# fakufaku/diffusion-separation

Hardware: AMD Instinct MI355X
Metric: separated utterances/sec (4 s, 8 kHz, 2-spk, N=30 PC steps) (higher is better)
Workload: dtype f16; 1 GPU; configs[1]: 2-spk N=30 PC sampler (+1 ald2 corrector step), batch=16 x 4.0 s @ 8 kHz per GPU and step, NCSN++ nf=64 random-init, 60 NFE/step; 4 consecutive steps (batches) in flight per GPU; batch_per_gpu=16, samples=32000, N=30, corrector_steps=1, nf=64, graph=True, batches_in_flight=4

## Files before the change

### diffusion-separation_amd/csrc/stft.hip

```cpp
#include <math.h>

#include <string.h>

#include <type_traits>
#include <vector>

#include "common.h"

#define DS_MAXC 4

long ds_stft_fwd_offset(int n_fft) { return ((long)3 * n_fft + 63) & ~63L; }
long ds_stft_inv_offset(int n_fft) { return ds_stft_fwd_offset(n_fft) + 512L * 512L; }
long ds_stft_ffrag_offset(int n_fft) { return ds_stft_inv_offset(n_fft) + 512L * 512L; }
constexpr long DS_STFT_FFRAG_FLOATS = 2L * 16 * 32 * 64 * 8 / 2;
long ds_stft_ifrag_offset(int n_fft) { return ds_stft_ffrag_offset(n_fft) + DS_STFT_FFRAG_FLOATS; }
int ds_build_stft_table(int n_fft, float** dev_tab) {
  if (n_fft > 510 || n_fft % 2) { ds_set_error("stft: n_fft must be even and <= 510"); return 1; }
  const int bins = n_fft / 2 + 1;
  std::vector<float> t((size_t)ds_stft_ifrag_offset(n_fft) + DS_STFT_FFRAG_FLOATS, 0.f);
  for (int n = 0; n < n_fft; ++n) {
    const double a = 2.0 * M_PI * (double)n / (double)n_fft;
    t[n] = (float)cos(a);
    t[n_fft + n] = (float)sin(a);
    t[2 * n_fft + n] = (float)(0.5 * (1.0 - cos(a)));
  }
  float* fw = t.data() + ds_stft_fwd_offset(n_fft);
  float* iv = t.data() + ds_stft_inv_offset(n_fft);
  for (int k = 0; k < bins; ++k)
    for (int n = 0; n < n_fft; ++n) {
      const double a = 2.0 * M_PI * (double)(((long)k * n) % n_fft) / (double)n_fft;
      fw[(size_t)k * 512 + n] = (float)cos(a);
      fw[(size_t)(256 + k) * 512 + n] = (float)(-sin(a));
      const double cj = (k == 0 || k == bins - 1) ? 1.0 : 2.0;
      const double wn = 0.5 * (1.0 - cos(2.0 * M_PI * (double)n / (double)n_fft)) / (double)n_fft;
      iv[(size_t)n * 512 + k] = (float)(wn * cj * cos(a));
      iv[(size_t)n * 512 + 256 + k] = (k == 0 || k == bins - 1) ? 0.f : (float)(-wn * cj * sin(a));
    }
  {
    bf16_t* fr = reinterpret_cast<bf16_t*>(t.data() + ds_stft_ffrag_offset(n_fft));
    const size_t part = (size_t)16 * 32 * 64 * 8;
    for (int rt = 0; rt < 16; ++rt)
      for (int ks = 0; ks < 32; ++ks)
        for (int lane = 0; lane < 64; ++lane)
          for (int j = 0; j < 8; ++j) {
            const int r = rt * 32 + (lane & 31), kb = r >> 1, im = r & 1, n = 16 * ks + 8 * (lane >> 5) + j;
            float v = 0.f;
            if (n < n_fft && kb < bins) {
              const double a = 2.0 * M_PI * (double)(((long)kb * n) % n_fft) / (double)n_fft;
              const double wn = 0.5 * (1.0 - cos(2.0 * M_PI * (double)n / (double)n_fft));
              v = (float)(wn * (im ? -sin(a) : cos(a)));
            }
            const bf16_t hi = f2bf(v);
            const size_t o = (((size_t)ks * 16 + rt) * 64 + lane) * 8 + j;
            fr[o] = hi;
            fr[part + o] = f2bf(v - bf2f(hi));
          }
  }
  {
    bf16_t* fr = reinterpret_cast<bf16_t*>(t.data() + ds_stft_ifrag_offset(n_fft));
    const size_t part = (size_t)16 * 32 * 64 * 8;
    for (int ct = 0; ct < 16; ++ct)
      for (int ks = 0; ks < 32; ++ks)
        for (int lane = 0; lane < 64; ++lane)
          for (int j = 0; j < 8; ++j) {
            const int n = ct * 32 + (lane & 31), K = 16 * ks + 8 * (lane >> 5) + j;
            const float v = iv[(size_t)n * 512 + K];
            const bf16_t hi = f2bf(v);
            const size_t o = (((size_t)ks * 16 + ct) * 64 + lane) * 8 + j;
            fr[o] = hi;
            fr[part + o] = f2bf(v - bf2f(hi));
          }
  }
  float* d = nullptr;
  DS_HIP(hipMalloc(&d, t.size() * sizeof(float)));
  DS_HIP(hipMemcpy(d, t.data(), t.size() * sizeof(float), hipMemcpyHostToDevice));
  *dev_tab = d;
  return 0;
}

__global__ __launch_bounds__(256) void stft_frame_kernel(const float* __restrict__ xt, const float* __restrict__ mix,
                                                         float* __restrict__ frames, int S, long Tlen, int n_fft,
                                                         int hop, int F, long rows, const float* __restrict__ tab) {
  const long i = (long)blockIdx.x * 256 + threadIdx.x;
  if (i >= rows * 128) return;
  const long row = i >> 7;
  const int n0 = (int)(i & 127) * 4;
  const int f = (int)(row % F);
  const long bc = row / F;
  const int NC = S + 1;
  const int ch = (int)(bc % NC);
  const long b = bc / NC;
  const float* src = (ch < S) ? xt + (b * S + ch) * Tlen : mix + b * Tlen;
  const long base = (long)f * hop - n_fft / 2;
  float v[4];
#pragma unroll
  for (int j = 0; j < 4; ++j) {
    const int n = n0 + j;
    const long idx = base + n;
    v[j] = (n < n_fft && idx >= 0 && idx < Tlen) ? src[idx] * tab[2 * n_fft + n] : 0.f;
  }
  *reinterpret_cast<float4*>(frames + row * 512 + n0) = make_float4(v[0], v[1], v[2], v[3]);
}

template <typename T>
__global__ __launch_bounds__(256) void stft_pack_kernel(const float* __restrict__ specT, T* __restrict__ y, int S,
                                                        int bins, int F, int W, int Cpad, long rows, float expo,
                                                        float factor, int shift, int B) {
  const long i = (long)blockIdx.x * 256 + threadIdx.x;
  const long total = (long)B * bins * W;
  if (i >= total) return;
  const int f = (int)(i % W);
  const int k = (int)((i / W) % bins);
  const long b = i / ((long)W * bins);
  const int NC = S + 1;
  float o[16];
#pragma unroll
  for (int j = 0; j < 16; ++j) o[j] = 0.f;
  if (f < F) {
#pragma unroll
    for (int ch = 0; ch < DS_MAXC; ++ch) {
      if (ch < NC) {
        const long row = (b * NC + ch) * F + f;
        const float re = specT[(long)k * rows + row], im = specT[(long)(256 + k) * rows + row];
        const float mag = sqrtf(re * re + im * im);
        float sc = 0.f;
        if (mag > 0.f) sc = (expo == 0.5f) ? (1.0f / sqrtf(mag)) : ((expo == 1.0f) ? 1.0f : powf(mag, expo - 1.0f));
        sc *= factor;
        float vr = re * sc, vi = im * sc;
        if (shift) { vr = 2.f * vr - 1.f; vi = 2.f * vi - 1.f; }
        if (ch == 0) { o[0] = vr; }
        if (ch == 1) { o[1] = vr; }
        if (ch == 2) { o[2] = vr; }
        if (ch == 3) { o[3] = vr; }
        const int q = NC + ch;
        if (q == 1) o[1] = vi; else if (q == 2) o[2] = vi; else if (q == 3) o[3] = vi; else if (q == 4) o[4] = vi;
        else if (q == 5) o[5] = vi; else if (q == 6) o[6] = vi; else if (q == 7) o[7] = vi;
      }
    }
  } else {
    const float pv = shift ? -1.f : 0.f;
#pragma unroll
    for (int j = 0; j < 16; ++j) o[j] = (j < 2 * NC) ? pv : 0.f;
  }
  T* dst = y + ((b * bins + k) * W + f) * Cpad;
  for (int c0 = 0; c0 < Cpad; c0 += 8) store8<T>(dst + c0, o + c0);
}

#ifdef ST_TIMING
__device__ unsigned long long g_st_dbg[16];
#define ST_DECL unsigned long long st_prev = __builtin_readcyclecounter();
#define ST_MARK(i) { const unsigned long long st_now = __builtin_readcyclecounter(); if (threadIdx.x == 0) atomicAdd(&g_st_dbg[i], st_now - st_prev); st_prev = st_now; }
extern "C" int diffsep_st_debug_read(unsigned long long* out, int reset) {
  (void)hipMemcpyFromSymbol(out, HIP_SYMBOL(g_st_dbg), sizeof(unsigned long long) * 16);
  if (reset) { unsigned long long z[16] = {0}; (void)hipMemcpyToSymbol(HIP_SYMBOL(g_st_dbg), z, sizeof(z)); }
  return 0;
}
#else
#define ST_DECL
#define ST_MARK(i)
#endif
constexpr int SF_PITCH = 272, SF_ROWS = 35, SF_CH = SF_ROWS * SF_PITCH, SF_NS = 32 * 128 + 382;
#ifndef SF_NW
#define SF_NW 4
#endif
constexpr int SF_NT = 64 * SF_NW, SF_RT = 8 / SF_NW;
template <int NC>
__global__ __launch_bounds__(SF_NT) void stft_fused_kernel(const float* __restrict__ xt, const float* __restrict__ mix,
                                                         bf16_t* __restrict__ y, long Tlen, int F, int W, float expo,
                                                         float factor, int shift, const uint4* __restrict__ dfrag) {
  extern __shared__ __attribute__((aligned(16))) char sm[];
  constexpr int S = NC - 1;
  const int tid = threadIdx.x, lane = tid & 63, wave = tid >> 6, l32 = lane & 31, h = lane >> 5;
  const int ntile = W >> 5;
  const int rh = blockIdx.x & 1, ft = (blockIdx.x >> 1) % ntile, b = (blockIdx.x >> 1) / ntile;
  const int f0 = ft * 32;
  const float pv = shift ? -1.f : 0.f;
  ST_DECL
  if (f0 >= F) {
    float o[8];
#pragma unroll
    for (int j = 0; j < 8; ++j) o[j] = j < 2 * NC ? pv : 0.f;
    for (int i = tid; i < 128 * 32; i += SF_NT) {
      const int kb = rh * 128 + (i >> 5), f = f0 + (i & 31);
      store8<bf16_t>(y + (((long)b * 256 + kb) * W + f) * 8, o);
    }
    return;
  }
  const long g0 = 128L * f0 - 255;
  constexpr int SF_NSP = (SF_NS + 7) & ~7;
  constexpr int NPAIR = NC * (SF_NSP / 2), NIT = (NPAIR + SF_NT - 1) / SF_NT, GRP = 9;
#pragma unroll
  for (int base = 0; base < NIT; base += GRP) {
    float v0[GRP], v1[GRP];
#pragma unroll
    for (int u = 0; u < GRP; ++u) {
      const int idx = tid + (base + u) * SF_NT;
      v0[u] = 0.f; v1[u] = 0.f;
      if (base + u < NIT && idx < NPAIR) {
        const int c = idx / (SF_NSP / 2), j = 2 * (idx - c * (SF_NSP / 2));
        const float* src = c < S ? xt + ((long)b * S + c) * Tlen : mix + (long)b * Tlen;
        const long t0 = g0 + j;
        if (t0 >= 0 && t0 < Tlen) v0[u] = src[t0];
        if (t0 + 1 >= 0 && t0 + 1 < Tlen) v1[u] = src[t0 + 1];
      }
    }
#pragma unroll
    for (int u = 0; u < GRP; ++u) {
      const int idx = tid + (base + u) * SF_NT;
      if (base + u < NIT && idx < NPAIR) {
        const int c = idx / (SF_NSP / 2), j = 2 * (idx - c * (SF_NSP / 2));
        const bf16_t h0 = f2bf(v0[u]), h1 = f2bf(v1[u]);
        const bf16_t l0 = f2bf(v0[u] - bf2f(h0)), l1 = f2bf(v1[u] - bf2f(h1));
        const int addr = 2 * j + 16 * (j >> 7);
        *reinterpret_cast<unsigned*>(sm + c * SF_CH + addr) = (unsigned)h0 | ((unsigned)h1 << 16);
        *reinterpret_cast<unsigned*>(sm + (NC + c) * SF_CH + addr) = (unsigned)l0 | ((unsigned)l1 << 16);
      }
    }
  }
  __syncthreads();
  ST_MARK(0)
  constexpr int RT = SF_RT;
  f32x16 acc[RT][NC];
#pragma unroll
  for (int t = 0; t < RT; ++t)
#pragma unroll
    for (int c = 0; c < NC; ++c)
#pragma unroll
      for (int e = 0; e < 16; ++e) acc[t][c][e] = 0.f;
  const int rt0 = rh * 8 + RT * wave;
  const uint4* ahi = dfrag + ((size_t)rt0 * 64 + lane);
  const uint4* alo = ahi + (size_t)16 * 32 * 64;
  constexpr int DEPTH = 3;
  uint4 a[DEPTH][RT][2];
#pragma unroll
  for (int d = 0; d < DEPTH; ++d)
#pragma unroll
    for (int t = 0; t < RT; ++t) { a[d][t][0] = ahi[((size_t)d * 16 + t) * 64]; a[d][t][1] = alo[((size_t)d * 16 + t) * 64]; }
  const char* bbase = sm + SF_PITCH * l32 + 16 * h;
#pragma unroll
  for (int ks = 0; ks < 32; ++ks) {
    const int n = 16 * ks;
    const int boff = 2 * n + 16 * (n >> 7);
    uint4 bh[NC], bl[NC];
#pragma unroll
    for (int c = 0; c < NC; ++c) {
      bh[c] = *reinterpret_cast<const uint4*>(bbase + c * SF_CH + boff);
      bl[c] = *reinterpret_cast<const uint4*>(bbase + (NC + c) * SF_CH + boff);
    }
    uint4 ah[RT], al[RT];
#pragma unroll
    for (int t = 0; t < RT; ++t) { ah[t] = a[ks % DEPTH][t][0]; al[t] = a[ks % DEPTH][t][1]; }
    if (ks + DEPTH < 32) {
#pragma unroll
      for (int t = 0; t < RT; ++t) {
        a[ks % DEPTH][t][0] = ahi[((size_t)(ks + DEPTH) * 16 + t) * 64];
        a[ks % DEPTH][t][1] = alo[((size_t)(ks + DEPTH) * 16 + t) * 64];
      }
    }
#pragma unroll
    for (int t = 0; t < RT; ++t)
#pragma unroll
      for (int c = 0; c < NC; ++c) {
        acc[t][c] = mfma_bf32(ah[t], bh[c], acc[t][c]);
        acc[t][c] = mfma_bf32(al[t], bh[c], acc[t][c]);
        acc[t][c] = mfma_bf32(ah[t], bl[c], acc[t][c]);
      }
  }
  ST_MARK(1)
  const int f = f0 + l32;
  auto epilogue = [&](auto MODE_) __attribute__((always_inline)) {
    constexpr int MODE = decltype(MODE_)::value;
#pragma unroll
    for (int t = 0; t < RT; ++t)
#pragma unroll
      for (int q = 0; q < 4; ++q)
#pragma unroll
        for (int kk = 0; kk < 2; ++kk) {
          const int kb = 16 * (rt0 + t) + 4 * q + 2 * h + kk;
          float o[8];
#pragma unroll
          for (int j = 0; j < 8; ++j) o[j] = 0.f;
#pragma unroll
          for (int c = 0; c < NC; ++c) {
            const float re = acc[t][c][4 * q + 2 * kk], im = acc[t][c][4 * q + 2 * kk + 1];
            const float m2 = fmaf(re, re, im * im);
            float sc;
            if constexpr (MODE == 0) sc = m2 > 0.f ? __builtin_amdgcn_rsqf(__builtin_amdgcn_sqrtf(m2)) : 0.f;
            else if constexpr (MODE == 1) sc = 1.f;
            else sc = m2 > 0.f ? powf(sqrtf(m2), expo - 1.0f) : 0.f;
            sc *= factor;
            float vr = re * sc, vi = im * sc;
            if (shift) { vr = fmaf(2.f, vr, -1.f); vi = fmaf(2.f, vi, -1.f); }
            o[c] = vr;
            o[NC + c] = vi;
          }
          if (f >= F) {
#pragma unroll
            for (int j = 0; j < 8; ++j) o[j] = j < 2 * NC ? pv : 0.f;
          }
          store8<bf16_t>(y + (((long)b * 256 + kb) * W + f) * 8, o);
        }
  };
  if (expo == 0.5f) epilogue(std::integral_constant<int, 0>{});
  else if (expo == 1.0f) epilogue(std::integral_constant<int, 1>{});
  else epilogue(std::integral_constant<int, 2>{});
  ST_MARK(2)
}

long ds_stft_workspace_bytes(int B, int S, long T, int n_fft, int hop) {
  const long F = 1 + (T + n_fft - hop) / hop;
  const long rows = (long)B * (S + 1) * F;
  return 2 * ((rows + 8) * 512 * 4 + 256);
}

int ds_launch_stft_pack(const float* xt, const float* mix, void* y, int B, int S, long T, int n_fft, int hop,
                        float exponent, float factor, int W, int Cpad, int shift, int dtype, const float* tab,
                        float* ws, hipStream_t st, int split) {
  DS_CHECK(S >= 1 && S + 1 <= DS_MAXC, "stft: num_sources must be in [1,3]");
  DS_CHECK(Cpad % 8 == 0 && Cpad >= 2 * (S + 1) && Cpad <= 16, "stft: bad channel padding");
  DS_CHECK(n_fft % 2 == 0 && n_fft >= 2 && n_fft <= 510 && hop >= 1, "stft: n_fft must be even and <= 510");
  const int F = 1 + (int)((T + n_fft - hop) / hop);
  DS_CHECK(W >= F, "stft: padded width smaller than the frame count");
  const int bins = n_fft / 2 + 1;
  if (dtype == DS_BF16 && n_fft == 510 && hop == 128 && Cpad == 8 && W % 32 == 0 && !(ds_default_opts() & DS_OPT_NO_STFT_FUSED)) {
    const uint4* dfrag = reinterpret_cast<const uint4*>(tab + ds_stft_ffrag_offset(n_fft));
    const unsigned nblk = (unsigned)(2 * (W / 32) * B);
#ifndef SF_LDS_MIN
#define SF_LDS_MIN 0
#endif
#define SFK(NC_)                                                                                                           \
  {                                                                                                                          \
    constexpr int LDS0_ = 2 * NC_ * SF_CH, LDS_ = LDS0_ > SF_LDS_MIN ? LDS0_ : SF_LDS_MIN;                                   \
    DS_FUNC_LDS_ONCE((stft_fused_kernel<NC_>), LDS_);                                                                        \
    hipLaunchKernelGGL((stft_fused_kernel<NC_>), dim3(nblk), dim3(SF_NT), LDS_, st, xt, mix, (bf16_t*)y, T, F, W, exponent, factor, shift, dfrag); \
    ds_set_last_conv_kernel("stft_fused_kernel<" #NC_ ">");                                                                  \
  }
    if (S == 1) SFK(2) else if (S == 2) SFK(3) else SFK(4)
#undef SFK
    DS_LAUNCH_CHECK();
    return 0;
  }
  const long rows = (long)B * (S + 1) * F;
  const long rows_p = (rows + 7) & ~7L;
  float* frames = ws;
  float* specT = ws + ((rows * 512 + 63) & ~63L);
  hipLaunchKernelGGL(stft_frame_kernel, dim3(cdiv(rows * 128, 256)), dim3(256), 0, st, xt, mix, frames, S, T, n_fft,
                     hop, F, rows, tab);
  DS_LAUNCH_CHECK();
  ConvArgs a;
  memset(&a, 0, sizeof(a));
  a.x = tab + ds_stft_fwd_offset(n_fft); a.ldx = 512; a.x_bs = 0;
  a.w = frames; a.w_bs = 0;
  a.y = specT; a.ldy = (int)rows_p; a.y_bs = 0;
  a.B = 1; a.H = 1; a.W = 512; a.Cin = 512; a.Cout = (int)rows; a.taps = 1; a.dtype = DS_F32; a.split = split; a.out_scale = 1.f;
  if (ds_launch_conv(a, st)) return 1;
  const long total = (long)B * bins * W;
  if (dtype == DS_F32)
    hipLaunchKernelGGL(stft_pack_kernel<float>, dim3(cdiv(total, 256)), dim3(256), 0, st, specT, (float*)y, S, bins, F,
                       W, Cpad, rows_p, exponent, factor, shift, B);
  else
    hipLaunchKernelGGL(stft_pack_kernel<bf16_t>, dim3(cdiv(total, 256)), dim3(256), 0, st, specT, (bf16_t*)y, S, bins,
                       F, W, Cpad, rows_p, exponent, factor, shift, B);
  DS_LAUNCH_CHECK();
  ds_set_last_conv_kernel(dtype == DS_F32 ? "stft_pack_kernel<f32>" : "stft_pack_kernel<" DS_HALF_NAME ">");
  return 0;
}

#define DS_FRAME_PITCH 512
template <typename T>
__global__ __launch_bounds__(256) void istft_unpack_kernel(const T* __restrict__ x, float* __restrict__ U, int S,
                                                           int bins, int F, int W, int Cpad, float expo, float factor,
                                                           long total, const float* __restrict__ ow,
                                                           const float* __restrict__ ob, const float* __restrict__ tdiv,
                                                           int ow_cin) {
  const long i = (long)blockIdx.x * 256 + threadIdx.x;
  if (i >= total) return;
  const int j = (int)(i & 255);
  const int f = (int)((i >> 8) % F);
  const long b = (i >> 8) / F;
  const float inv_fac = 1.0f / fabsf(factor);
  float v[8];
  if (j < bins) load8<T>(x + ((b * bins + j) * W + f) * Cpad, v);
  if (ow && j < bins) {
    float h[8];
#pragma unroll
    for (int k = 0; k < 8; ++k) h[k] = v[k];
    const float td = tdiv[b];
#pragma unroll
    for (int c = 0; c < 8; ++c) {
      float a = 0.f;
      if (c < 2 * S) {
#pragma unroll
        for (int k = 0; k < 8; ++k)
          if (k < ow_cin) a = fmaf(ow[c * ow_cin + k], h[k], a);
        a = a / td + ob[c];
      }
      v[c] = a;
    }
  }
#pragma unroll
  for (int s = 0; s < DS_MAXC - 1; ++s) {
    if (s < S) {
      float re = 0.f, im = 0.f;
      if (j < bins) {
        const float vr = v[s] * inv_fac, vi = v[S + s] * inv_fac;
        const float mag = sqrtf(vr * vr + vi * vi);
        float sc = 0.f;
        if (mag > 0.f) sc = (expo == 0.5f) ? mag : ((expo == 1.0f) ? 1.0f : powf(mag, 1.0f / expo - 1.0f));
        re = vr * sc;
        im = vi * sc;
      }
      float* row = U + ((b * S + s) * F + f) * 512;
      row[j] = re;
      row[256 + j] = im;
    }
  }
}

__global__ __launch_bounds__(256) void istft_ola_kernel(const float* __restrict__ frames, float* __restrict__ out,
                                                        long Tlen, int n_fft, int hop, int F,
                                                        const float* __restrict__ tab) {
  const long t = (long)blockIdx.x * 256 + threadIdx.x;
  const long bs = blockIdx.y;
  if (t >= Tlen) return;
  float v = 0.f;
  if (t < (long)hop * (F - 1)) {
    const long q = t + n_fft / 2;
    long f_hi = q / hop;
    if (f_hi > F - 1) f_hi = F - 1;
    long f_lo = (q - (n_fft - 1) + hop - 1) / hop;
    if (q - (n_fft - 1) <= 0) f_lo = 0;
    float num = 0.f, den = 0.f;
    for (long f = f_lo; f <= f_hi; ++f) {
      const int n = (int)(q - f * hop);
      const float w = tab[2 * n_fft + n];
      num += frames[(bs * F + f) * DS_FRAME_PITCH + n];
      den = fmaf(w, w, den);
    }
    v = num / den;
  }
  out[bs * Tlen + t] = v;
}

constexpr int SI_PITCH = 1040, SI_U = 32 * SI_PITCH, SI_SEG = 29 * 128;
#ifndef SI_NW
#define SI_NW 16
#endif
constexpr int SI_NT = 64 * SI_NW, SI_CT = 16 / SI_NW;
template <int NS, int EM>
__global__ __launch_bounds__(SI_NT, NS == 1 ? 2 : 1) void istft_fused_kernel(const bf16_t* __restrict__ x, float* __restrict__ out, int S,
                                                             long Tlen, int F, int W, int ld, float expo, float factor,
                                                             const float* __restrict__ ow, const float* __restrict__ ob,
                                                             const float* __restrict__ tdiv, int ow_cin,
                                                             const uint4* __restrict__ dfrag, const float* __restrict__ tab,
                                                             int nseg) {
  extern __shared__ __attribute__((aligned(16))) char sm[];
  constexpr int SRC = 2 * SI_U;
  const int tid = threadIdx.x, lane = tid & 63, wave = tid >> 6, l32 = lane & 31, h = lane >> 5;
  const int nsg = S / NS;
  const int seg = blockIdx.x % nseg, s0 = ((blockIdx.x / nseg) % nsg) * NS, b = blockIdx.x / (nseg * nsg);
  const int g0 = 29 * seg, fA = g0 - 1;
  ST_DECL
  {
    const float inv_fac = 1.0f / fabsf(factor);
    float wre[NS][8], wim[NS][8], bre[NS], bim[NS];
#pragma unroll
    for (int ns = 0; ns < NS; ++ns) {
      const int s = s0 + ns;
#pragma unroll
      for (int k = 0; k < 8; ++k) {
        wre[ns][k] = (ow && k < ow_cin) ? ow[s * ow_cin + k] : (k == s ? 1.f : 0.f);
        wim[ns][k] = (ow && k < ow_cin) ? ow[(S + s) * ow_cin + k] : (k == S + s ? 1.f : 0.f);
      }
      bre[ns] = ow ? ob[s] : 0.f;
      bim[ns] = ow ? ob[S + s] : 0.f;
    }
    const float inv_td = ow ? 1.0f / tdiv[b] : 1.f;
    constexpr int BG = SI_NT / 32;
    const int r = tid & 31, f = fA + r;
    const bool fok = f >= 0 && f < F;
    char* u = sm + r * SI_PITCH;
#pragma unroll
    for (int base = 0; base < 256 / BG; base += 8) {
      uint4 raw[8];
#pragma unroll
      for (int q = 0; q < 8; ++q) {
        const int kb = (tid >> 5) + BG * (base + q);
        raw[q] = fok ? *reinterpret_cast<const uint4*>(x + (((long)b * 256 + kb) * W + f) * ld) : make_uint4(0, 0, 0, 0);
      }
#pragma unroll
      for (int q = 0; q < 8; ++q) {
        const int kb = (tid >> 5) + BG * (base + q);
        float v[8];
        v[0] = h_lo(raw[q].x); v[1] = h_hi(raw[q].x); v[2] = h_lo(raw[q].y); v[3] = h_hi(raw[q].y);
        v[4] = h_lo(raw[q].z); v[5] = h_hi(raw[q].z); v[6] = h_lo(raw[q].w); v[7] = h_hi(raw[q].w);
#pragma unroll
        for (int ns = 0; ns < NS; ++ns) {
          float re = 0.f, im = 0.f;
          if (fok) {
            float ar = 0.f, ai = 0.f;
#pragma unroll
            for (int k = 0; k < 8; ++k) { ar = fmaf(wre[ns][k], v[k], ar); ai = fmaf(wim[ns][k], v[k], ai); }
            if (ow) { ar = fmaf(ar, inv_td, bre[ns]); ai = fmaf(ai, inv_td, bim[ns]); }
            const float vr = ar * inv_fac, vi = ai * inv_fac;
            const float m2 = fmaf(vr, vr, vi * vi);
            float sc;
            if constexpr (EM == 0) sc = __builtin_amdgcn_sqrtf(m2);
            else if constexpr (EM == 1) sc = 1.f;
            else sc = m2 > 0.f ? powf(sqrtf(m2), 1.0f / expo - 1.0f) : 0.f;
            re = vr * sc;
            im = vi * sc;
          }
          const bf16_t rh_ = f2bf(re), ih_ = f2bf(im);
          char* un = u + ns * SRC;
          *reinterpret_cast<bf16_t*>(un + 2 * kb) = rh_;
          *reinterpret_cast<bf16_t*>(un + 2 * (256 + kb)) = ih_;
          *reinterpret_cast<bf16_t*>(un + SI_U + 2 * kb) = f2bf(re - bf2f(rh_));
          *reinterpret_cast<bf16_t*>(un + SI_U + 2 * (256 + kb)) = f2bf(im - bf2f(ih_));
        }
      }
    }
  }
  __syncthreads();
  ST_MARK(4)
  constexpr int CT = SI_CT;
  f32x16 acc[NS][CT];
#pragma unroll
  for (int ns = 0; ns < NS; ++ns)
#pragma unroll
    for (int c = 0; c < CT; ++c)
#pragma unroll
      for (int e = 0; e < 16; ++e) acc[ns][c][e] = 0.f;
  const uint4* bhi = dfrag + ((size_t)(CT * wave) * 64 + lane);
  const uint4* blo = bhi + (size_t)16 * 32 * 64;
#ifndef SI_DEPTH
#define SI_DEPTH 3
#endif
  constexpr int DEPTH = SI_DEPTH;
  uint4 bf[DEPTH][CT][2];
#pragma unroll
  for (int d = 0; d < DEPTH; ++d)
#pragma unroll
    for (int c = 0; c < CT; ++c) { bf[d][c][0] = bhi[((size_t)d * 16 + c) * 64]; bf[d][c][1] = blo[((size_t)d * 16 + c) * 64]; }
  const char* abase = sm + SI_PITCH * l32 + 16 * h;
#pragma unroll
  for (int ks = 0; ks < 32; ++ks) {
    uint4 ah[NS], al[NS];
#pragma unroll
    for (int ns = 0; ns < NS; ++ns) {
      ah[ns] = *reinterpret_cast<const uint4*>(abase + ns * SRC + 32 * ks);
      al[ns] = *reinterpret_cast<const uint4*>(abase + ns * SRC + SI_U + 32 * ks);
    }
    uint4 bh_[CT], bl_[CT];
#pragma unroll
    for (int c = 0; c < CT; ++c) { bh_[c] = bf[ks % DEPTH][c][0]; bl_[c] = bf[ks % DEPTH][c][1]; }
    if (ks + DEPTH < 32) {
#pragma unroll
      for (int c = 0; c < CT; ++c) {
        bf[ks % DEPTH][c][0] = bhi[((size_t)(ks + DEPTH) * 16 + c) * 64];
        bf[ks % DEPTH][c][1] = blo[((size_t)(ks + DEPTH) * 16 + c) * 64];
      }
    }
#pragma unroll
    for (int c = 0; c < CT; ++c)
#pragma unroll
      for (int ns = 0; ns < NS; ++ns) {
        acc[ns][c] = mfma_bf32(ah[ns], bh_[c], acc[ns][c]);
        acc[ns][c] = mfma_bf32(al[ns], bh_[c], acc[ns][c]);
        acc[ns][c] = mfma_bf32(ah[ns], bl_[c], acc[ns][c]);
      }
  }
  ST_MARK(5)
  __syncthreads();
  float* w2 = reinterpret_cast<float*>(sm) + 4 * SI_SEG;
  for (int i = tid; i < 512; i += SI_NT) { const float w = i < 510 ? tab[2 * 510 + i] : 0.f; w2[i] = w * w; }
#pragma unroll
  for (int ns = 0; ns < NS; ++ns) {
    float* mine = reinterpret_cast<float*>(sm + ns * SRC) + (wave * CT / 4) * SI_SEG;
#pragma unroll
    for (int c = 0; c < CT; ++c) {
      const int n = 32 * (CT * wave + c) + l32;
#pragma unroll
      for (int e = 0; e < 16; ++e) {
        const int r = 8 * (e >> 2) + 4 * h + (e & 3);
        const int p = 128 * r + n - 383;
        if (n < 510 && p >= 0 && p < SI_SEG) mine[p] = acc[ns][c][e];
      }
    }
  }
  __syncthreads();
  ST_MARK(6)
  for (int i = tid; i < SI_SEG; i += SI_NT) {
    const long t = 128L * g0 + i;
    if (t >= Tlen) break;
    if (t < 128L * (F - 1)) {
      const long q = t + 255;
      long f_hi = q / 128;
      if (f_hi > F - 1) f_hi = F - 1;
      long f_lo = (q - 509 + 127) / 128;
      if (q - 509 <= 0) f_lo = 0;
      float den = 0.f;
      for (long f = f_lo; f <= f_hi; ++f) den += w2[(int)(q - f * 128)];
      const float inv_den = 1.0f / den;
#pragma unroll
      for (int ns = 0; ns < NS; ++ns) {
        const float* ola = reinterpret_cast<const float*>(sm + ns * SRC);
        float num = 0.f;
#pragma unroll
        for (int w = 0; w < 4; ++w) {
          const int n = 128 * w + ((i + 383) & 127), r = (i + 383 - n) >> 7;
          if (n < 510 && r >= 0 && r < 32) num += ola[w * SI_SEG + i];
        }
        out[((long)b * S + s0 + ns) * Tlen + t] = num * inv_den;
      }
    } else {
#pragma unroll
      for (int ns = 0; ns < NS; ++ns) out[((long)b * S + s0 + ns) * Tlen + t] = 0.f;
    }
  }
  ST_MARK(7)
}

long ds_istft_workspace_bytes(int B, int S, long T, int n_fft, int hop) {
  const long F = 1 + (T + n_fft - hop) / hop;
  return 2 * ((long)B * S * F * 512 * 4 + 256);
}

int ds_launch_istft(const void* x, float* out, int B, int S, long T, int n_fft, int hop, float exponent, float factor,
                    int W, int Cpad, int dtype, const float* tab, float* ws, hipStream_t st, int split, const float* ow,
                    const float* ob, const float* tdiv, int ow_cin) {
  DS_CHECK(n_fft % 2 == 0 && n_fft <= 510, "istft: n_fft must be even and <= 510");
  DS_CHECK(!ow || (ob && tdiv), "istft: the fused output layer needs its bias and the per-entry divisor");
  DS_CHECK(S >= 1 && S <= DS_MAXC - 1 && Cpad >= 2 * S && Cpad % 8 == 0 && 2 * S <= 8, "istft: bad source / channel count");
  const int F = 1 + (int)((T + n_fft - hop) / hop);
  DS_CHECK(W >= F, "istft: padded width smaller than the frame count");
  DS_CHECK(!ow || (ow_cin >= 2 * S && ow_cin <= 8), "istft: the fused output layer needs 2 * num_sources <= ow_cin <= 8 input channels");
  const int bins = n_fft / 2 + 1;
  if (dtype == DS_BF16 && n_fft == 510 && hop == 128 && Cpad % 8 == 0 && (!ow || ow_cin <= 8) && !(ds_default_opts() & DS_OPT_NO_STFT_FUSED)) {
    const uint4* dfrag = reinterpret_cast<const uint4*>(tab + ds_stft_ifrag_offset(n_fft));
    const int nseg = (int)cdiv(T, (long)SI_SEG);
    constexpr int LDS1 = 2 * SI_U;
    static_assert(4 * SI_SEG * 4 + 512 * 4 <= LDS1, "the four per-wave copies of the segment and the squared window fit the U planes");
#define ISK(NS_, EM_)                                                                                                                     \
  {                                                                                                                                          \
    DS_FUNC_LDS_ONCE((istft_fused_kernel<NS_, EM_>), NS_ * LDS1);                                                                            \
    hipLaunchKernelGGL((istft_fused_kernel<NS_, EM_>), dim3((unsigned)(B * (S / NS_) * nseg)), dim3(SI_NT), NS_ * LDS1, st, (const bf16_t*)x, out, \
                       S, T, F, W, Cpad, exponent, factor, ow, ob, tdiv, ow_cin, dfrag, tab, nseg);                                       \
    ds_set_last_conv_kernel("istft_fused_kernel<" #NS_ "," #EM_ ">");                                                                         \
  }
    const int em = exponent == 0.5f ? 0 : (exponent == 1.0f ? 1 : 2);
#ifdef SI_NS1
    if (false) {}
#else
    if (S == 2) { if (em == 0) ISK(2, 0) else if (em == 1) ISK(2, 1) else ISK(2, 2) }
#endif
    else { if (em == 0) ISK(1, 0) else if (em == 1) ISK(1, 1) else ISK(1, 2) }
#undef ISK
    DS_LAUNCH_CHECK();
    return 0;
  }
  const long rows = (long)B * S * F;
  float* U = ws;
  float* frames = ws + ((rows * 512 + 63) & ~63L);
  const long total = (long)B * F * 256;
  if (dtype == DS_F32)
    hipLaunchKernelGGL(istft_unpack_kernel<float>, dim3(cdiv(total, 256)), dim3(256), 0, st, (const float*)x, U, S, bins,
                       F, W, Cpad, exponent, factor, total, ow, ob, tdiv, ow_cin);
  else
    hipLaunchKernelGGL(istft_unpack_kernel<bf16_t>, dim3(cdiv(total, 256)), dim3(256), 0, st, (const bf16_t*)x, U, S,
                       bins, F, W, Cpad, exponent, factor, total, ow, ob, tdiv, ow_cin);
  DS_LAUNCH_CHECK();
  ConvArgs a;
  memset(&a, 0, sizeof(a));
  a.x = U; a.ldx = 512; a.x_bs = 0;
  a.w = tab + ds_stft_inv_offset(n_fft); a.w_bs = 0;
  a.y = frames; a.ldy = DS_FRAME_PITCH; a.y_bs = 0;
  a.B = 1; a.H = 1; a.W = (int)rows; a.Cin = 512; a.Cout = 512; a.taps = 1; a.dtype = DS_F32; a.split = split; a.out_scale = 1.f;
  if (ds_launch_conv(a, st)) return 1;
  dim3 g2((unsigned)cdiv(T, 256), (unsigned)(B * S));
  hipLaunchKernelGGL(istft_ola_kernel, g2, dim3(256), 0, st, frames, out, T, n_fft, hop, F, tab);
  DS_LAUNCH_CHECK();
  ds_set_last_conv_kernel("istft_ola_kernel");
  return 0;
}
```

Before: 74.75 utterances/s.

## Exploit iSTFT basis symmetry to halve fused iSTFT matrix work

Rebuilds the inverse-DFT fragment table so that only the first half of the output samples (n<256) is computed, with separate real and imaginary partial sums. The mirrored samples (510-n) are then recovered as the sum rather than the difference of the two accumulators, using the cos/sin symmetry of the basis. The block size now scales with the number of sources (8 waves per source) instead of a fixed 16 waves. The B-fragment prefetch and the window load are hoisted ahead of the spectrum preparation. This is meant to halve the MFMA and B-fragment traffic per block. It depends on the symmetry holding for n_fft=510 and on the new mirror write-back being correct.

```diff
diff --git a/diffusion-separation_amd/csrc/stft.hip b/diffusion-separation_amd/csrc/stft.hip
--- a/diffusion-separation_amd/csrc/stft.hip
+++ b/diffusion-separation_amd/csrc/stft.hip
@@ -14,10 +14,11 @@
 long ds_stft_ffrag_offset(int n_fft) { return ds_stft_inv_offset(n_fft) + 512L * 512L; }
 constexpr long DS_STFT_FFRAG_FLOATS = 2L * 16 * 32 * 64 * 8 / 2;
 long ds_stft_ifrag_offset(int n_fft) { return ds_stft_ffrag_offset(n_fft) + DS_STFT_FFRAG_FLOATS; }
+constexpr long DS_STFT_IFRAG_FLOATS = 2L * 16 * 2 * 8 * 64 * 8 / 2;
 int ds_build_stft_table(int n_fft, float** dev_tab) {
   if (n_fft > 510 || n_fft % 2) { ds_set_error("stft: n_fft must be even and <= 510"); return 1; }
   const int bins = n_fft / 2 + 1;
-  std::vector<float> t((size_t)ds_stft_ifrag_offset(n_fft) + DS_STFT_FFRAG_FLOATS, 0.f);
+  std::vector<float> t((size_t)ds_stft_ifrag_offset(n_fft) + DS_STFT_IFRAG_FLOATS, 0.f);
   for (int n = 0; n < n_fft; ++n) {
     const double a = 2.0 * M_PI * (double)n / (double)n_fft;
     t[n] = (float)cos(a);
@@ -58,18 +59,19 @@
   }
   {
     bf16_t* fr = reinterpret_cast<bf16_t*>(t.data() + ds_stft_ifrag_offset(n_fft));
-    const size_t part = (size_t)16 * 32 * 64 * 8;
-    for (int ct = 0; ct < 16; ++ct)
-      for (int ks = 0; ks < 32; ++ks)
-        for (int lane = 0; lane < 64; ++lane)
-          for (int j = 0; j < 8; ++j) {
-            const int n = ct * 32 + (lane & 31), K = 16 * ks + 8 * (lane >> 5) + j;
-            const float v = iv[(size_t)n * 512 + K];
-            const bf16_t hi = f2bf(v);
-            const size_t o = (((size_t)ks * 16 + ct) * 64 + lane) * 8 + j;
-            fr[o] = hi;
-            fr[part + o] = f2bf(v - bf2f(hi));
-          }
+    const size_t part = (size_t)16 * 2 * 8 * 64 * 8;
+    for (int ks = 0; ks < 16; ++ks)
+      for (int pr = 0; pr < 2; ++pr)
+        for (int ct = 0; ct < 8; ++ct)
+          for (int lane = 0; lane < 64; ++lane)
+            for (int j = 0; j < 8; ++j) {
+              const int n = ct * 32 + (lane & 31), K = 16 * ks + 8 * (lane >> 5) + j;
+              const float v = pr ? -iv[(size_t)n * 512 + 256 + K] : iv[(size_t)n * 512 + K];
+              const bf16_t hi = f2bf(v);
+              const size_t o = ((((size_t)ks * 2 + pr) * 8 + ct) * 64 + lane) * 8 + j;
+              fr[o] = hi;
+              fr[part + o] = f2bf(v - bf2f(hi));
+            }
   }
   float* d = nullptr;
   DS_HIP(hipMalloc(&d, t.size() * sizeof(float)));
@@ -443,12 +445,9 @@
 }
 
 constexpr int SI_PITCH = 1040, SI_U = 32 * SI_PITCH, SI_SEG = 29 * 128;
-#ifndef SI_NW
-#define SI_NW 16
-#endif
-constexpr int SI_NT = 64 * SI_NW, SI_CT = 16 / SI_NW;
+constexpr int si_nt(int ns) { return 64 * 8 * ns; }
 template <int NS, int EM>
-__global__ __launch_bounds__(SI_NT, NS == 1 ? 2 : 1) void istft_fused_kernel(const bf16_t* __restrict__ x, float* __restrict__ out, int S,
+__global__ __launch_bounds__(si_nt(NS), NS == 1 ? 2 : 1) void istft_fused_kernel(const bf16_t* __restrict__ x, float* __restrict__ out, int S,
                                                              long Tlen, int F, int W, int ld, float expo, float factor,
                                                              const float* __restrict__ ow, const float* __restrict__ ob,
                                                              const float* __restrict__ tdiv, int ow_cin,
@@ -456,11 +455,25 @@
                                                              int nseg) {
   extern __shared__ __attribute__((aligned(16))) char sm[];
   constexpr int SRC = 2 * SI_U;
+  constexpr int SI_NT = si_nt(NS);
   const int tid = threadIdx.x, lane = tid & 63, wave = tid >> 6, l32 = lane & 31, h = lane >> 5;
   const int nsg = S / NS;
   const int seg = blockIdx.x % nseg, s0 = ((blockIdx.x / nseg) % nsg) * NS, b = blockIdx.x / (nseg * nsg);
   const int g0 = 29 * seg, fA = g0 - 1;
   ST_DECL
+  const int ct = wave & 7, ns = wave >> 3;
+  const uint4* bhi = dfrag + ((size_t)ct * 64 + lane);
+  const uint4* blo = bhi + (size_t)16 * 2 * 8 * 64;
+#ifndef SI_DEPTH
+#define SI_DEPTH 3
+#endif
+  constexpr int DEPTH = SI_DEPTH;
+  uint4 bf[DEPTH][2][2];
+#pragma unroll
+  for (int d = 0; d < DEPTH; ++d)
+#pragma unroll
+    for (int pr = 0; pr < 2; ++pr) { bf[d][pr][0] = bhi[((size_t)d * 2 + pr) * 8 * 64]; bf[d][pr][1] = blo[((size_t)d * 2 + pr) * 8 * 64]; }
+  const float wpre = tid < 510 ? tab[2 * 510 + tid] : 0.f;
   {
     const float inv_fac = 1.0f / fabsf(factor);
     float wre[NS][8], wim[NS][8], bre[NS], bim[NS];
@@ -523,69 +536,45 @@
   }
   __syncthreads();
   ST_MARK(4)
-  constexpr int CT = SI_CT;
-  f32x16 acc[NS][CT];
-#pragma unroll
-  for (int ns = 0; ns < NS; ++ns)
-#pragma unroll
-    for (int c = 0; c < CT; ++c)
-#pragma unroll
-      for (int e = 0; e < 16; ++e) acc[ns][c][e] = 0.f;
-  const uint4* bhi = dfrag + ((size_t)(CT * wave) * 64 + lane);
-  const uint4* blo = bhi + (size_t)16 * 32 * 64;
-#ifndef SI_DEPTH
-#define SI_DEPTH 3
-#endif
-  constexpr int DEPTH = SI_DEPTH;
-  uint4 bf[DEPTH][CT][2];
-#pragma unroll
-  for (int d = 0; d < DEPTH; ++d)
-#pragma unroll
-    for (int c = 0; c < CT; ++c) { bf[d][c][0] = bhi[((size_t)d * 16 + c) * 64]; bf[d][c][1] = blo[((size_t)d * 16 + c) * 64]; }
-  const char* abase = sm + SI_PITCH * l32 + 16 * h;
-#pragma unroll
-  for (int ks = 0; ks < 32; ++ks) {
-    uint4 ah[NS], al[NS];
-#pragma unroll
-    for (int ns = 0; ns < NS; ++ns) {
-      ah[ns] = *reinterpret_cast<const uint4*>(abase + ns * SRC + 32 * ks);
-      al[ns] = *reinterpret_cast<const uint4*>(abase + ns * SRC + SI_U + 32 * ks);
-    }
-    uint4 bh_[CT], bl_[CT];
-#pragma unroll
-    for (int c = 0; c < CT; ++c) { bh_[c] = bf[ks % DEPTH][c][0]; bl_[c] = bf[ks % DEPTH][c][1]; }
-    if (ks + DEPTH < 32) {
-#pragma unroll
-      for (int c = 0; c < CT; ++c) {
-        bf[ks % DEPTH][c][0] = bhi[((size_t)(ks + DEPTH) * 16 + c) * 64];
-        bf[ks % DEPTH][c][1] = blo[((size_t)(ks + DEPTH) * 16 + c) * 64];
-      }
-    }
-#pragma unroll
-    for (int c = 0; c < CT; ++c)
-#pragma unroll
-      for (int ns = 0; ns < NS; ++ns) {
-        acc[ns][c] = mfma_bf32(ah[ns], bh_[c], acc[ns][c]);
-        acc[ns][c] = mfma_bf32(al[ns], bh_[c], acc[ns][c]);
-        acc[ns][c] = mfma_bf32(ah[ns], bl_[c], acc[ns][c]);
-      }
+  f32x16 accA, accB;
+#pragma unroll
+  for (int e = 0; e < 16; ++e) { accA[e] = 0.f; accB[e] = 0.f; }
+  const char* abase = sm + ns * SRC + SI_PITCH * l32 + 16 * h;
+#pragma unroll
+  for (int ks = 0; ks < 16; ++ks) {
+    const uint4 rh_ = *reinterpret_cast<const uint4*>(abase + 32 * ks), rl_ = *reinterpret_cast<const uint4*>(abase + SI_U + 32 * ks);
+    const uint4 ih_ = *reinterpret_cast<const uint4*>(abase + 512 + 32 * ks), il_ = *reinterpret_cast<const uint4*>(abase + SI_U + 512 + 32 * ks);
+    const uint4 ah_ = bf[ks % DEPTH][0][0], al_ = bf[ks % DEPTH][0][1], bh_ = bf[ks % DEPTH][1][0], bl_ = bf[ks % DEPTH][1][1];
+    if (ks + DEPTH < 16) {
+#pragma unroll
+      for (int pr = 0; pr < 2; ++pr) {
+        bf[ks % DEPTH][pr][0] = bhi[((size_t)(ks + DEPTH) * 2 + pr) * 8 * 64];
+        bf[ks % DEPTH][pr][1] = blo[((size_t)(ks + DEPTH) * 2 + pr) * 8 * 64];
+      }
+    }
+    accA = mfma_bf32(rh_, ah_, accA);
+    accB = mfma_bf32(ih_, bh_, accB);
+    accA = mfma_bf32(rl_, ah_, accA);
+    accB = mfma_bf32(il_, bh_, accB);
+    accA = mfma_bf32(rh_, al_, accA);
+    accB = mfma_bf32(ih_, bl_, accB);
   }
   ST_MARK(5)
   __syncthreads();
   float* w2 = reinterpret_cast<float*>(sm) + 4 * SI_SEG;
-  for (int i = tid; i < 512; i += SI_NT) { const float w = i < 510 ? tab[2 * 510 + i] : 0.f; w2[i] = w * w; }
-#pragma unroll
-  for (int ns = 0; ns < NS; ++ns) {
-    float* mine = reinterpret_cast<float*>(sm + ns * SRC) + (wave * CT / 4) * SI_SEG;
-#pragma unroll
-    for (int c = 0; c < CT; ++c) {
-      const int n = 32 * (CT * wave + c) + l32;
-#pragma unroll
-      for (int e = 0; e < 16; ++e) {
-        const int r = 8 * (e >> 2) + 4 * h + (e & 3);
-        const int p = 128 * r + n - 383;
-        if (n < 510 && p >= 0 && p < SI_SEG) mine[p] = acc[ns][c][e];
-      }
+  if (tid < 512) w2[tid] = wpre * wpre;
+  {
+    float* copies = reinterpret_cast<float*>(sm + ns * SRC);
+    const int n = 32 * ct + l32, m = 510 - n;
+    float* direct = copies + (n >> 7) * SI_SEG;
+    float* mirror = copies + (m >> 7) * SI_SEG;
+    const bool has_mirror = n >= 1 && n <= 254;
+#pragma unroll
+    for (int e = 0; e < 16; ++e) {
+      const int r = 8 * (e >> 2) + 4 * h + (e & 3);
+      const int p = 128 * r + n - 383, pm = 128 * r + m - 383;
+      if (p >= 0 && p < SI_SEG) direct[p] = accA[e] - accB[e];
+      if (has_mirror && pm >= 0 && pm < SI_SEG) mirror[pm] = accA[e] + accB[e];
     }
   }
   __syncthreads();
@@ -644,7 +633,7 @@
 #define ISK(NS_, EM_)                                                                                                                     \
   {                                                                                                                                          \
     DS_FUNC_LDS_ONCE((istft_fused_kernel<NS_, EM_>), NS_ * LDS1);                                                                            \
-    hipLaunchKernelGGL((istft_fused_kernel<NS_, EM_>), dim3((unsigned)(B * (S / NS_) * nseg)), dim3(SI_NT), NS_ * LDS1, st, (const bf16_t*)x, out, \
+    hipLaunchKernelGGL((istft_fused_kernel<NS_, EM_>), dim3((unsigned)(B * (S / NS_) * nseg)), dim3(si_nt(NS_)), NS_ * LDS1, st, (const bf16_t*)x, out, \
                        S, T, F, W, Cpad, exponent, factor, ow, ob, tdiv, ow_cin, dfrag, tab, nseg);                                       \
     ds_set_last_conv_kernel("istft_fused_kernel<" #NS_ "," #EM_ ">");                                                                         \
   }
```

After: 74.97 utterances/s, median of 6. Within noise of the previous version (+0.3%).
